# lyltc1/ZebraPose

Measured on AMD Instinct MI355X. Metric: 256x256 crops/sec (R34 DeepLabv3 inference bs=32, forward + code->vertex decode), higher is better.
Workload: dtype f32; 1 GPU; configs[1]: ResNet34+DeepLabv3 inference bs=32 on 1xMI355X, synthetic 256x256 crops, 16-bit code head, on-device decode; model=BinaryCodeNet_Deeplab(34, 16, 2, concat=True), global_batch=32, per_gpu_batch=32, input=256x256, parallelism=replicas1, precision=fp32, launch=hipgraph, fp32_engine=two-plane fp16 split fp32 (ZP_F32H2; range-guarded, full-range x3 fallback), correspondences_last_step=227718

## Files before the change

zebrapose_amd/csrc/zp_conv.hip:

```cpp
#include <type_traits>
#include "zp_common.h"
#include "zp_conv_kern.h"
#include "zp_conv3.h"

namespace zp {

__device__ uint4 g_zero_page[8];

template <typename T, int WC, int WP, int NWP, bool BNR = false>
__device__ __forceinline__ void conv_epilogue(const zp_conv_args& A, const zp_conv_sub& S, f32x4 (&acc)[WC][WP],
                                              const int p0, const int c0, const int wc, const int wp, const int lane,
                                              const int M, const int GHW, const int bx, const int zi,
                                              const int nz, unsigned* rflag = nullptr, float* red = nullptr) {
  int pn[WP], poy[WP], pox[WP];
  bool pok[WP];
  {
    const int pw0 = p0 + wp * 16 * WP + (lane & 15);
    int n = pw0 / GHW, rr = pw0 - n * GHW;
    int gy = rr / A.GW, gx = rr - gy * A.GW;
    const bool fast = A.GW % 16 == 0;
#pragma unroll
    for (int j = 0; j < WP; ++j) {
      const int p = pw0 + j * 16;
      pok[j] = p < M;
// ... 1975 lines not shown
}

extern "C" long long zp_conv2d_split_ws(const zp_conv_args* a) {
  if (!a || (a->dtype != ZP_F32X3 && a->dtype != ZP_F32H2)) return 0;
  const int ns = conv3_nsplit(*a);
  return ns > 1 ? (long long)ns * a->nsub * a->N * a->GH * a->GW * a->Cout * 4 : 0;
}

extern "C" int zp_conv_tuning(int key, int value) {
  int* g = nullptr;
  switch (key) {
    case 0: g = &g_tc256_min_blocks; break;
    case 1: g = &g_conv_flags; break;
    case 2: g = &g_strip_c64; break;
    case 6: g = &g_quad_min_blocks; break;
    case 3:
    case 4:
    case 5: return wgrad_tuning(key, value);
    case 7: return conv3_strip_mode(value);
    case 8: return conv3_min_blocks(value);
    case 9: return conv3_splitk_mode(value);
    case 10: return conv3w_mode(value);
    case 11: return conv3w_min_blocks(value);
    case 12: return conv3w_splitk_mode(value);
    case 13: return conv3w_acc_mode(value);
    case 14: return conv3w_tp128_mode(value);
    case 15: return bn_fused_mode(value);
    case 16: return conv3_subint_mode(value);
    case 17: return conv3w_subint_mode(value);
    case 18: return conv3w_mf32_mode(value);
    case 19: return conv3_pipe_st_mode(value);
    case 20: return stem_wgs_mode(value);
    case 21: return conv3w_pfb_mode(value);
    default: return -1;
  }
  const int old = *g;
  *g = value;
  return old;
}
```

zebrapose_amd/csrc/zp_conv3.h:

```cpp
#pragma once
#include "zp_common.h"

namespace zp {
int conv3_tc(const zp_conv_args& a);
int conv3_tp(const zp_conv_args& a, int tc);
bool conv3_strip_ok(const zp_conv_args& a, int tc);
int conv3_strip_mode(int v);
int conv3_min_blocks(int v);
int conv3_splitk_mode(int v);
int conv3_nsplit(const zp_conv_args& a);
int conv3_subint_mode(int v);
int conv3_pipe_st_mode(int v);
int stem_wgs_mode(int v);
int conv3w_pfb_mode(int v);
int wgrad_tuning(int key, int v);
int conv3_launch(const zp_conv_args& a, hipStream_t st, int flags, const zp_head_args* head = nullptr);
struct conv_taps;
bool conv3w_ok(const zp_conv_args& a);
int conv3w_mode(int v);
int conv3w_min_blocks(int v);
void conv3w_launch(const zp_conv_args& a, const conv_taps& tg, hipStream_t st, int flags, float* ws, int nsplit);
int conv3w_splitk(const zp_conv_args& a);
int conv3w_splitk_mode(int v);
int conv3w_tp(const zp_conv_args& a);
int conv3w_tp_head(const zp_conv_args& a);
int conv3w_acc_mode(int v);
int conv3w_tp128_mode(int v);
int conv3w_subint_mode(int v);
int conv3w_mf32_mode(int v);
bool conv3w_mf32_on();
void conv3w32_launch(const zp_conv_args& a, const conv_taps& tg, hipStream_t st, int flags, bool str);
void conv3w_head_launch(const zp_conv_args& a, const conv_taps& tg, const zp_head_args& h, hipStream_t st, int flags);
}
```

zebrapose_amd/csrc/zp_conv3.hip:

```cpp
#include <stdlib.h>
#include "zp_conv_kern.h"
#include "zp_conv3.h"

namespace zp {

__device__ __forceinline__ void block_barrier() {
  __builtin_amdgcn_s_barrier();
  asm volatile("" ::: "memory");
}

template <int NPL, int WC, int WP>
__device__ __forceinline__ void conv3_epilogue(const zp_conv_args& A, const zp_conv_sub& S, f32x4 (&acc)[WC][WP],
                                               const int p0, const int c0, const int wc, const int wp,
                                               const int lane, const int M, const int GHW, const int flags,
                                               unsigned* rflag) {
  using SP = SplitF32<NPL>;
  const int lr = lane & 15;
  bool bad = false;
  int pn[WP], poy[WP], pox[WP];
  bool pok[WP];
#pragma unroll
  for (int j = 0; j < WP; ++j) {
    const int p = p0 + wp * 16 * WP + j * 16 + lr;
    pok[j] = p < M;
    const int pp = pok[j] ? p : 0;
    const int n = pp / GHW, rr = pp - n * GHW;
    const int gy = rr / A.GW, gx = rr - gy * A.GW;
    pn[j] = n;
    poy[j] = gy * S.oys + S.oyo;
    pox[j] = gx * S.oxs + S.oxo;
  }
  const long psy = (long)A.N * S.OH * S.OW * S.ldy;
  const long psr = (long)A.N * S.OH * S.OW * A.ldr;
  if constexpr (WC % 2 == 0) {
    const bool paired = A.out_mode == ZP_OUT_NHWC && S.ldy % 8 == 0 && S.cy0 % 8 == 0 && A.Cout % 32 == 0 &&
// ... 315 lines not shown
  static_assert(WP == 4 || WP == 8, "pixel fragments per wave");
  __shared__ uint4 lds[ST * UNITS * 64];
  static_assert(ST * UNITS * 1024 <= 160 * 1024, "LDS");
  static_assert(((NPL - 1) * NT + WC + 3) * 1024 < 65536, "ds_read immediate range");
  int tb = (int)blockIdx.z / nsplit;
  const int kz = (int)blockIdx.z - tb * nsplit;
  const int tid = threadIdx.x, lane = tid & 63;
  const int wid = __builtin_amdgcn_readfirstlane(tid >> 6);
  const int wc = wid / NWP, wp = wid % NWP;
  const int GHW = A.GH * A.GW;
  const int M = A.N * GHW;
  int bx = blockIdx.x, by = blockIdx.y;
  const int total = gridDim.x * gridDim.y;
  if ((flags & 1048576) && nsplit == 1 && A.nsub > 1 && (total & 7) == 0) {
    const int gid = blockIdx.x + gridDim.x * (blockIdx.y + gridDim.y * blockIdx.z);
    const int q = gid >> 3;
    tb = q % A.nsub;
    const int tile = (gid & 7) * (total >> 3) + q / A.nsub;
    bx = tile / gridDim.y;
    by = tile - bx * gridDim.y;
  } else if (flags & 2) {
    const int bid = blockIdx.x + gridDim.x * blockIdx.y;
    const int lin = (total & 7) ? bid : (bid & 7) * (total >> 3) + (bid >> 3);
    bx = lin / gridDim.y;
    by = lin - bx * gridDim.y;
  }
  tb = __builtin_amdgcn_readfirstlane(tb);
  const zp_conv_sub& S = A.sub[tb];
  const int p0 = bx * TP, c0 = by * TC;
  const int CB = A.Cin / 32;
  const int ny = TG.ny[tb], nx = TG.nx[tb], dty = TG.dty[tb], dtx = TG.dtx[tb];
  const int nK_all = S.ntaps * CB;
  const int ks0 = (int)((long)kz * nK_all / nsplit);
  const int nK = (int)((long)(kz + 1) * nK_all / nsplit) - ks0;
  const int lr = lane & 15, lk = (lane >> 4) * 8;
  const unsigned psx_b = (unsigned)((long)A.N * A.IH * A.IW * A.ldx * 2);
  const unsigned psw_b = (unsigned)((long)A.w_rows * A.k_pad * 2);

  unsigned ubase[TPW], uym[TPW], uxm[TPW];
#pragma unroll
  for (int k = 0; k < TPW; ++k) {
    const int t = wid + NW * k;
    ubase[k] = 0u;
    uym[k] = uxm[k] = 0u;
    if (t >= NT) continue;
    if (t < NTW) {
      ubase[k] = (unsigned)(((long)(c0 + t * 16 + lr) * A.k_pad + lk) * 2);
    } else {
      const int m = p0 + (t - NTW) * 16 + lr;
      const bool ok = m < M;
      const int mm = ok ? m : 0;
      const int n = mm / GHW, rr = mm - n * GHW;
      const int gy = rr / A.GW, gx = rr - gy * A.GW;
      const int y0 = gy * A.sy, x0 = gx * A.sx;
      ubase[k] = (unsigned)(((((long)n * A.IH + y0) * A.IW + x0) * A.ldx + A.cx0 + lk) * 2);
      unsigned ym = 0, xm = 0;
      for (int q = 0; q < ny; ++q) ym |= (unsigned)((unsigned)(y0 + TG.ty0[tb] + q * dty) < (unsigned)A.IH) << q;
      for (int q = 0; q < nx; ++q) xm |= (unsigned)((unsigned)(x0 + TG.tx0[tb] + q * dtx) < (unsigned)A.IW) << q;
      uym[k] = ok ? ym : 0u;
      uxm[k] = xm;
    }
  }
#if defined(__HIP_DEVICE_COMPILE__)
  const __amdgpu_buffer_rsrc_t xrsrc = __builtin_amdgcn_make_buffer_rsrc((void*)A.x, (short)0, (int)TG.x_bytes, 0x00020000);
  const __amdgpu_buffer_rsrc_t wrsrc = __builtin_amdgcn_make_buffer_rsrc((void*)S.w, (short)0, (int)TG.w_bytes[tb], 0x00020000);
#endif
  int w_cb = ks0 / S.ntaps, w_t = ks0 - (ks0 / S.ntaps) * S.ntaps;
  int w_tyi = w_t / nx, w_txi = w_t - (w_t / nx) * nx;
  const int step_x = dtx * A.ldx * 2, step_y = dty * A.IW * A.ldx * 2;
  int act_off = ((TG.ty0[tb] * A.IW + TG.tx0[tb]) * A.ldx) * 2 + w_tyi * step_y + w_txi * step_x + w_cb * 64;
  int w_koff = (w_t * A.Cin + w_cb * 32) * 2;
  const int cin2 = A.Cin * 2;
  const bool abl_dma = flags & 4096, abl_mfma = flags & 8192;
  auto issue = [&](int ks, int stage) {
    unsigned voff[TPW];
#pragma unroll
    for (int k = 0; k < TPW; ++k) {
      const bool w = wid + NW * k < NTW;
      const bool ok = (uym[k] >> w_tyi) & (uxm[k] >> w_txi) & 1u;
      voff[k] = w ? ubase[k] : (ok ? ubase[k] + (unsigned)act_off : 0x80000000u);
    }
#if defined(__HIP_DEVICE_COMPILE__)
#pragma unroll
    for (int k = 0; k < TPW; ++k) {
      const int t = wid + NW * k;
      if (t >= NT) continue;
#pragma unroll
      for (int pl = 0; pl < NPL; ++pl) {
        auto* d = (__attribute__((address_space(3))) void*)&lds[(stage * UNITS + pl * NT + t) * 64];
        if (t < NTW) __builtin_amdgcn_raw_ptr_buffer_load_lds(wrsrc, d, 16, voff[k], pl * psw_b + w_koff, 0, 0);
        else __builtin_amdgcn_raw_ptr_buffer_load_lds(xrsrc, d, 16, voff[k], pl * psx_b, 0, 0);
      }
    }
#endif
    (void)ks;
    ++w_t;
    w_koff += cin2;
    act_off += step_x;
    if (++w_txi == nx) {
      w_txi = 0;
      act_off += step_y - nx * step_x;
      if (++w_tyi == ny) {
        w_tyi = 0;
        w_t = 0;
        ++w_cb;
        act_off += 64 - ny * step_y;
        w_koff = w_cb * 64;
      }
    }
  };

  constexpr int A2C = PIPE ? WC : 1, A2P = PIPE ? WP : 1;
  f32x4 acc[WC][WP], acc2[A2C][A2P];
#pragma unroll
  for (int i = 0; i < WC; ++i)
#pragma unroll
    for (int j = 0; j < WP; ++j) acc[i][j] = (f32x4){0.f, 0.f, 0.f, 0.f};
#pragma unroll
  for (int i = 0; i < A2C; ++i)
#pragma unroll
    for (int j = 0; j < A2P; ++j) acc2[i][j] = (f32x4){0.f, 0.f, 0.f, 0.f};

  const unsigned l0 = lds_addr(lds) + (unsigned)lane * 16u;
  unsigned abase[ST], bbase[ST];
#pragma unroll
  for (int s = 0; s < ST; ++s) {
    abase[s] = l0 + (unsigned)(s * UNITS + wc * WC) * 1024u;
    bbase[s] = l0 + (unsigned)(s * UNITS + NTW + wp * WP) * 1024u;
  }
  const int awo = (wc * WC) * 64 + lane, bwo = (NTW + wp * WP) * 64 + lane;
  auto read_a = [&](auto s_c, uint4 (&af)[NPL][WC]) {
    constexpr int s = decltype(s_c)::value;
    static_for<NPL>([&](auto p_c) {
      constexpr int p = decltype(p_c)::value;
      static_for<WC>([&](auto i) {
        if constexpr (PIPE) af[p][i] = lds[(s * UNITS + p * NT + i) * 64 + awo];
        else af[p][i] = ds_read16<(p * NT + i) * 1024>(abase[s]);
      });
    });
  };
  auto read_b = [&](auto s_c, auto j0_c, auto j1_c, uint4 (&bfr)[NPL][WP]) {
    constexpr int s = decltype(s_c)::value, J0 = decltype(j0_c)::value, J1 = decltype(j1_c)::value;
// ... 66 lines not shown
      constexpr int s = decltype(s_c)::value;
      const bool more = ks + ST - 1 < nK;
      if (more && !abl_dma) issue(ks + ST - 1, (s + ST - 1) % ST);
      uint4 af[NPL][WC], bfr[NPL][WP];
      read_a(s_c, af);
      read_b(s_c, J0c{}, JHc{}, bfr);
      asm volatile("s_waitcnt lgkmcnt(0)" ::: "memory");
      __builtin_amdgcn_sched_barrier(0);
      read_b(s_c, JHc{}, JWc{}, bfr);
      auto wait_next = [&]() {
        if (more && !abl_dma) vm_wait<GRP * (ST - 2)>();
        else vm_wait<0>();
      };
      if (pingpong) {
        wait_next();
        block_barrier();
        __builtin_amdgcn_sched_barrier(0);
      }
      if (flags & 4) __builtin_amdgcn_s_setprio(1);
      mfmas_part(J0c{}, JHc{}, af, bfr);
      __builtin_amdgcn_sched_barrier(0);
      asm volatile("s_waitcnt lgkmcnt(0)" ::: "memory");
      __builtin_amdgcn_sched_barrier(0);
      mfmas_part(JHc{}, JWc{}, af, bfr);
      __builtin_amdgcn_sched_barrier(0);
      if (flags & 4) __builtin_amdgcn_s_setprio(0);
      if (!pingpong) wait_next();
      block_barrier();
      __builtin_amdgcn_sched_barrier(0);
    };
    using I0 = std::integral_constant<int, 0>;
    using I1 = std::integral_constant<int, 1>;
    using I2 = std::integral_constant<int, 2>;
    issue(0, 0);
    if (ST == 3 && nK > 1) {
      issue(1, 1);
      vm_wait<GRP>();
    } else {
      vm_wait<0>();
    }
    block_barrier();
    __builtin_amdgcn_sched_barrier(0);
    if (pingpong && wid >= 4) block_barrier();
    if constexpr (ST == 3) {
      for (int ks = 0; ks < nK; ks += 3) {
        step(I0{}, ks);
        if (ks + 1 >= nK) break;
        step(I1{}, ks + 1);
        if (ks + 2 >= nK) break;
        step(I2{}, ks + 2);
      }
    } else {
      for (int ks = 0; ks < nK; ks += 2) {
        step(I0{}, ks);
        if (ks + 1 >= nK) break;
        step(I1{}, ks + 1);
      }
    }
    if (pingpong && wid < 4) block_barrier();
  } else {
    uint4 fa0[NPL][WC], fb0[NPL][WP], fa1[NPL][WC], fb1[NPL][WP];
    int issued = 0;
    for (int q = 0; q < ST; ++q)
      if (q < nK) {
        issue(q, q);
        ++issued;
      }
// ... 358 lines not shown
    sg->W = W;
    sg->TR = TR;
    sg->SW = SW;
    sg->SR = SR;
    sg->ty0 = ty0;
    sg->dty = dty;
    sg->tx0 = tx0;
    sg->dtx = dtx;
    sg->pad = pad;
  }
  return true;
}

static int g_splitk = 1;
static int g_subint = -1;
int conv3_subint_mode(int v) {
  const int old = g_subint;
  g_subint = v;
  return old;
}

static int g_pipe_st = -1;
int conv3_pipe_st_mode(int v) {
  const int old = g_pipe_st;
  g_pipe_st = v;
  return old;
}
static int conv3_pipe_st() {
  static const int env = getenv("ZP_CONV3_PIPE_ST") ? atoi(getenv("ZP_CONV3_PIPE_ST")) : 2;
  const int v = g_pipe_st >= 0 ? g_pipe_st : env;
  return v == 3 || v == 4 ? v : 2;
}

int conv3_splitk_mode(int v) {
  const int old = g_splitk;
  g_splitk = v;
  return old;
}

int conv3_nsplit(const zp_conv_args& a) {
  if (!g_splitk || a.out_mode != ZP_OUT_NHWC || a.nsub < 1) return 1;
  const int tc = conv3_tc(a);
  if (tc == 256) return conv3w_splitk(a);
  const long blocks = (long)ceil_div((long)a.N * a.GH * a.GW, conv3_tp(a, tc)) * ceil_div(a.Cout, tc) * a.nsub;
  int nK = 1 << 30;
  for (int s = 0; s < a.nsub; ++s) nK = min(nK, a.sub[s].ntaps * (a.Cin / 32));
  if (blocks >= 256) return 1;
  int ns = 1;
  while (ns < 16 && blocks * ns * 2 <= 512 && nK / (ns * 2) >= (a.nsub > 1 ? 4 : 8)) ns *= 2;
  return ns;
}

template <int NPL>
static void conv3_dispatch(const zp_conv_args& a, const conv_taps& tg, int tc, hipStream_t st, int fl) {
  if (tc == 256) {
    const int ns = a.stats ? conv3w_splitk(a) : 1;
    conv3w_launch(a, tg, st, fl, (float*)a.stats, ns);
    if (ns > 1) {
      const long total = (long)a.N * a.GH * a.GW * ((a.Cout + 3) / 4);
      const int blocks = (int)(total + 255) / 256 < 8192 ? (int)((total + 255) / 256) : 8192;
      hipLaunchKernelGGL((k_splitk_epi<NPL>), dim3(blocks, a.nsub), dim3(256), 0, st, a, (const float*)a.stats, ns,
                         tg.rflag);
    }
    return;
  }
  const int ns = a.stats ? conv3_nsplit(a) : 1;
// ... 48 lines not shown
  }
}

int conv3_launch(const zp_conv_args& a, hipStream_t st, int fl, const zp_head_args* head) {
  const int npl = a.dtype == ZP_F32H2 ? 2 : 3;
  ZP_CHECK_ARG(a.Cin > 0 && a.Cin % 32 == 0, "zp_conv2d: split fp32 needs Cin %% 32 == 0 (got %d; the stem runs in f32 "
               "with out_mode ZP_OUT_NHWC_X3 / _H2)", a.Cin);
  ZP_CHECK_ARG(a.ldx >= a.cx0 + a.Cin && a.cx0 % 8 == 0 && a.ldx % 8 == 0, "zp_conv2d: bad ldx/cx0");
  ZP_CHECK_ARG(a.k_pad % 32 == 0, "zp_conv2d: k_pad %d not a multiple of 32", a.k_pad);
  ZP_CHECK_ARG(a.out_mode == ZP_OUT_NHWC || a.out_mode == ZP_OUT_HEAD_NCHW,
               "zp_conv2d: split fp32 writes split NHWC (ZP_OUT_NHWC) or the f32 head (ZP_OUT_HEAD_NCHW)");
  const int tc = conv3_tc(a);
  ZP_CHECK_ARG(a.w_rows % tc == 0 && a.w_rows >= a.Cout, "zp_conv2d: w_rows %d", a.w_rows);
  for (int s = 0; s < a.nsub; ++s) {
    const zp_conv_sub& S = a.sub[s];
    ZP_CHECK_ARG(S.w && S.y, "zp_conv2d: sub %d null w/y", s);
    ZP_CHECK_ARG(S.ntaps >= 1 && S.ntaps <= ZP_MAX_TAPS && (long)S.ntaps * a.Cin <= a.k_pad,
                 "zp_conv2d: sub %d ntaps %d / k_pad %d", s, S.ntaps, a.k_pad);
    if (a.out_mode == ZP_OUT_NHWC)
      ZP_CHECK_ARG(S.ldy >= S.cy0 + a.Cout && S.cy0 % 4 == 0 && S.ldy % 4 == 0, "zp_conv2d: bad ldy/cy0");
    else
      ZP_CHECK_ARG(S.y2 || a.Cout == 1, "zp_conv2d: head needs y2");
    ZP_CHECK_ARG(S.OH == a.sub[0].OH && S.OW == a.sub[0].OW, "zp_conv2d: split-fp32 subs must share the output shape");
  }
  if (a.res) ZP_CHECK_ARG(a.ldr >= a.cr0 + a.Cout && a.cr0 % 4 == 0 && a.ldr % 4 == 0, "zp_conv2d: bad residual ld");
  conv_taps tg{};
  const long long xb = (long long)npl * a.N * a.IH * a.IW * a.ldx * 2;
  const long long wb = (long long)npl * a.w_rows * a.k_pad * 2;
  ZP_CHECK_ARG(xb < (1ll << 31) && wb < (1ll << 31),
               "zp_conv2d: split input (%lld B) / weights (%lld B) must stay below 2 GiB per launch (split the batch)",
               xb, wb);
  tg.x_bytes = (unsigned)xb;
  tg.rflag = npl == 2 ? range_flag() : nullptr;
  for (int s = 0; s < a.nsub; ++s) {
    const zp_conv_sub& S = a.sub[s];
    tg.w_bytes[s] = (unsigned)wb;
    int nx = 1;
    while (nx < S.ntaps && S.ty[nx] == S.ty[0]) ++nx;
    const int ny = S.ntaps / nx;
    tg.ny[s] = ny;
    tg.nx[s] = nx;
    tg.ty0[s] = S.ty[0];
    tg.tx0[s] = S.tx[0];
    tg.dty[s] = ny > 1 ? S.ty[nx] - S.ty[0] : 0;
    tg.dtx[s] = nx > 1 ? S.tx[1] - S.tx[0] : 0;
    bool grid = ny * nx == S.ntaps && ny <= 32 && nx <= 32;
    for (int t = 0; grid && t < S.ntaps; ++t)
      grid = S.ty[t] == tg.ty0[s] + (t / nx) * tg.dty[s] && S.tx[t] == tg.tx0[s] + (t % nx) * tg.dtx[s];
    ZP_CHECK_ARG(grid, "zp_conv2d: sub %d taps must form a (row x column) grid of at most 32 x 32, rows outer", s);
  }
  if (head) {
    const zp_head_args& h = *head;
    ZP_CHECK_ARG(tc == 256 && a.Cout == 256 && a.nsub == 1 && npl == 2,
                 "zp_conv2d_head: not a fused-head geometry (zp_conv2d_head_ok)");
    ZP_CHECK_ARG(h.w && h.mask && (h.code || h.cout == 1) && h.cout >= 1 && h.cout <= 32, "zp_conv2d_head: bad head");
    ZP_CHECK_ARG(h.C2 >= 0 && h.C2 % 32 == 0 && h.k_pad % 8 == 0 && h.k_pad >= a.Cout + h.C2 && h.k_pad <= 504,
                 "zp_conv2d_head: C2 %d / k_pad %d", h.C2, h.k_pad);
    ZP_CHECK_ARG(h.C2 == 0 || (h.x2 && h.ldx2 % 8 == 0 && h.cx20 % 8 == 0 && h.ldx2 >= h.cx20 + h.C2),
                 "zp_conv2d_head: x2 layout");
    conv3w_head_launch(a, tg, h, st, fl);
    ZP_LAUNCH_CHECK("zp_conv2d_head");
    return ZP_OK;
  }
  if (npl == 2) conv3_dispatch<2>(a, tg, tc, st, fl);
  else conv3_dispatch<3>(a, tg, tc, st, fl);
  ZP_LAUNCH_CHECK("zp_conv2d split-f32");
  return ZP_OK;
}


bool conv3_strip_ok(const zp_conv_args& a, int tc) { return conv3_strip(a, tc, nullptr); }

}
```

zebrapose_amd/csrc/zp_conv3w.hip:

```cpp
#include "zp_conv_kern.h"
#include "zp_conv3.h"

namespace zp {

constexpr int ACC_FLUSH = 0;
constexpr int ACC_SA = 1;
constexpr int ACC_PS = 2;
constexpr int ACC_FS = 3;
constexpr int ACC_P2 = 4;

__device__ __forceinline__ void wbarrier() {
  __builtin_amdgcn_s_barrier();
  asm volatile("" ::: "memory");
}

#ifdef ZP_STAMP
constexpr int ZP_STAMP_WAVES = 1 << 17;
__device__ unsigned long long zp_stamp_buf[ZP_STAMP_WAVES * 8];
#endif

template <int ABL, int DM, bool HEAD, bool SGB = false, bool PF = false, bool BF = false, bool STR = false,
          int NUM = ACC_FLUSH, int TPX = 256, bool PFB = false>
__global__ void __launch_bounds__(512) k_conv3w(const zp_conv_args A, const conv_taps TG, const int flags,
                                                const zp_head_args H, float* __restrict__ ws, const int nsplit) {
  constexpr int NPL = 2;
  constexpr int TC = 256, TP = TPX;
  static_assert(TP == 256 || TP == 128, "pixel tile");
  static_assert(TP == 256 || (!HEAD && !BF && DM == 1), "the 256 x 128 tile: plain epilogue, default DMA order");
  constexpr bool SA = NUM == ACC_SA || NUM == ACC_PS || NUM == ACC_FS;
  constexpr bool P2 = NUM == ACC_P2;
  static_assert(!P2 || (TPX == 128 && !HEAD), "the persistent correction accumulator: 256 x 128 tiles");
  static_assert(!PFB || (STR && !P2 && NUM == ACC_FLUSH && TPX == 256), "pixel-fragment prefetch: the strip tile");
  constexpr int NTW = TC / 16, NT = (TC + TP) / 16;
  constexpr int UNITS = NPL * NT;
// ... 9 lines not shown
  __shared__ uint4 lds[LDSU * 64];
  static_assert(LDSU * 1024 <= 160 * 1024, "LDS");
  static_assert(((NPL - 1) * NT + NT - 1) * 1024 < 65536, "ds_read immediate range");
  int tb = (int)blockIdx.z / nsplit;
  const int kz = (int)blockIdx.z - tb * nsplit;
  const int tid = threadIdx.x, lane = tid & 63;
  const int wid = __builtin_amdgcn_readfirstlane(tid >> 6);
  const int wc = wid >> 2, wp = wid & 3;
  const int GHW = A.GH * A.GW;
  const int M = A.N * GHW;
  int bx = blockIdx.x, by = blockIdx.y;
  const int total = gridDim.x * gridDim.y;
  if ((flags & 32768) && nsplit == 1 && A.nsub > 1 && (total & 7) == 0) {
    const int gid = blockIdx.x + gridDim.x * (blockIdx.y + gridDim.y * blockIdx.z);
    const int q = gid >> 3;
    tb = q % A.nsub;
    const int tile = (gid & 7) * (total >> 3) + q / A.nsub;
    bx = tile / gridDim.y;
    by = tile - bx * gridDim.y;
  } else if (flags & 2) {
    const int bid = blockIdx.x + gridDim.x * blockIdx.y;
    const int lin = (total & 7) ? bid : (bid & 7) * (total >> 3) + (bid >> 3);
    bx = lin / gridDim.y;
    by = lin - bx * gridDim.y;
  }
  tb = __builtin_amdgcn_readfirstlane(tb);
  const zp_conv_sub& S = A.sub[tb];
  const int p0 = bx * TP, c0 = by * TC;
  const int CB = A.Cin / 32;
  const int ny = TG.ny[tb], nx = TG.nx[tb], dty = TG.dty[tb], dtx = TG.dtx[tb];
  const int nK_all = S.ntaps * CB;
  const int kq = STR ? nx : 1, nq = nK_all / kq;
  const int ks0 = (int)((long)kz * nq / nsplit) * kq;
  const int nK = (int)((long)(kz + 1) * nq / nsplit) * kq - ks0;
  const int lr = lane & 15, lk = (lane >> 4) * 8;
  const unsigned psx_b = (unsigned)((long)A.N * A.IH * A.IW * A.ldx * 2);
  const unsigned psw_b = (unsigned)((long)A.w_rows * A.k_pad * 2);

  unsigned ubase[TPW], uym[TPW], uxm[TPW];
#pragma unroll
  for (int k = 0; k < TPW; ++k) {
    const int t = wid + 8 * k;
    uym[k] = uxm[k] = 0u;
    if (t < NTW) {
      ubase[k] = (unsigned)(((long)(c0 + t * 16 + lr) * A.k_pad + lk) * 2);
    } else {
      const int m = p0 + (t - NTW) * 16 + lr;
      const bool ok = m < M;
      const int mm = ok ? m : 0;
      const int n = mm / GHW, rr = mm - n * GHW;
      const int gy = rr / A.GW, gx = rr - gy * A.GW;
      const int y0 = gy * A.sy, x0 = gx * A.sx;
      ubase[k] = (unsigned)(((((long)n * A.IH + y0) * A.IW + x0) * A.ldx + A.cx0 + lk) * 2);
      unsigned ym = 0, xm = 0;
      for (int q = 0; q < ny; ++q) ym |= (unsigned)((unsigned)(y0 + TG.ty0[tb] + q * dty) < (unsigned)A.IH) << q;
      for (int q = 0; q < nx; ++q) xm |= (unsigned)((unsigned)(x0 + TG.tx0[tb] + q * dtx) < (unsigned)A.IW) << q;
      uym[k] = ok ? ym : 0u;
      uxm[k] = xm;
    }
  }
  int nsp = 16, SW = 0, sh0 = 0;
  unsigned sbase[3], sym[3];
  int sj[WP];
  if constexpr (STR) {
    const int sx0 = min(TG.tx0[tb], TG.tx0[tb] + (nx - 1) * dtx);
    sh0 = TG.tx0[tb] - sx0;
    SW = A.GW + (nx - 1) * (dtx < 0 ? -dtx : dtx);
    const int TR = TP / A.GW;
    nsp = (TR * SW + 15) >> 4;
    const int n = p0 / GHW, oy0 = (p0 - n * GHW) / A.GW;
#pragma unroll
    for (int k = 0; k < 3; ++k) {
      const int sp = (wid + 8 * k) * 16 + lr;
      const int r = sp / SW, c = sp - (sp / SW) * SW;
      const int ix = c + sx0, iyb = oy0 + r + TG.ty0[tb];
      unsigned ym = 0;
      for (int q = 0; q < ny; ++q) ym |= (unsigned)((unsigned)(iyb + q * dty) < (unsigned)A.IH) << q;
      sym[k] = (r < TR && (unsigned)ix < (unsigned)A.IW) ? ym : 0u;
      sbase[k] = (unsigned)(((((long)n * A.IH + iyb) * A.IW + ix) * A.ldx + A.cx0 + lk) * 2);
    }
#pragma unroll
    for (int j = 0; j < WP; ++j) {
      const int q = wp * 16 * WP + j * 16 + lr;
      sj[j] = (q / A.GW) * SW + q % A.GW;
    }
  }
#if defined(__HIP_DEVICE_COMPILE__)
  const __amdgpu_buffer_rsrc_t xrsrc = __builtin_amdgcn_make_buffer_rsrc((void*)A.x, (short)0, (int)TG.x_bytes, 0x00020000);
  const __amdgpu_buffer_rsrc_t wrsrc = __builtin_amdgcn_make_buffer_rsrc((void*)S.w, (short)0, (int)TG.w_bytes[tb], 0x00020000);
#endif
  const int t0 = ks0 % S.ntaps;
  int w_cb = ks0 / S.ntaps, w_tyi = t0 / nx, w_txi = t0 - (t0 / nx) * nx;
  const int step_x = dtx * A.ldx * 2, step_y = dty * A.IW * A.ldx * 2;
  int act_off = ((TG.ty0[tb] * A.IW + TG.tx0[tb]) * A.ldx) * 2 + w_tyi * step_y + w_txi * step_x + w_cb * 64;
  int w_koff = (t0 * A.Cin + w_cb * 32) * 2;
  const int cin2 = A.Cin * 2;
  struct DmaStep {
    unsigned voff[TPW];
    int koff;
  };
  unsigned pf_sink = 0;
  const bool pf_hi = (lane >> 5) & 1;
  constexpr int PFT = TPW - 1;
  const unsigned pf_base = pf_hi ? ubase[PFT] : ubase[2], pf_ym = pf_hi ? uym[PFT] : uym[2], pf_xm = pf_hi ? uxm[PFT] : uxm[2];
  const unsigned pf_plane = ((lane >> 4) & 1) ? psx_b : 0u;
  auto prep = [&](DmaStep& d) {
#pragma unroll
    for (int k = 0; k < TPW; ++k) {
      bool ok = (uym[k] >> w_tyi) & (uxm[k] >> w_txi) & 1u;
      if constexpr (ABL == 6) ok = ok && w_txi == 0;
      d.voff[k] = k < 2 ? ubase[k] : (ok ? ubase[k] + (unsigned)act_off : 0x80000000u);
    }
#if defined(__HIP_DEVICE_COMPILE__)
    if constexpr (PF) {
      const bool ok = w_tyi == 0 && w_txi == 0 && w_cb + 1 < CB && (pf_ym & pf_xm & 1u);
      const unsigned vo = ok ? pf_base + (unsigned)(act_off + 64) + pf_plane : 0x80000000u;
      pf_sink = __builtin_amdgcn_raw_buffer_load_b32(xrsrc, vo, 0, 0);
    }
#endif
    d.koff = w_koff;
    w_koff += cin2;
    act_off += step_x;
    if (++w_txi == nx) {
      w_txi = 0;
      act_off += step_y - nx * step_x;
      if (++w_tyi == ny) {
        w_tyi = 0;
        ++w_cb;
        act_off += 64 - ny * step_y;
        w_koff = w_cb * 64;
      }
    }
  };
  auto piece = [&](auto q_c, int stage, const DmaStep& d) {
    constexpr int q = decltype(q_c)::value, k = q / 2, pl = q % 2;
    if constexpr ((ABL == 4 && k < 2) || (ABL == 5 && k >= 2)) return;
    if constexpr (STR && k >= 2) return;
    const int t = wid + 8 * k;
#if defined(__HIP_DEVICE_COMPILE__)
    auto* dst = (__attribute__((address_space(3))) void*)&lds[(stage * ASTG + pl * APL + t) * 64];
    if constexpr (k < 2) __builtin_amdgcn_raw_ptr_buffer_load_lds(wrsrc, dst, 16, d.voff[k], pl * psw_b + d.koff, 0, 0);
    else __builtin_amdgcn_raw_ptr_buffer_load_lds(xrsrc, dst, 16, d.voff[k], pl * psx_b, 0, 0);
#else
    (void)t; (void)stage; (void)d;
#endif
  };
  auto issue = [&](int stage) {
    DmaStep d;
    prep(d);
    static_for<2 * TPW>([&](auto q_c) { piece(q_c, stage, d); });
  };
  int g_cb = ks0 / S.ntaps, g_tyi = (ks0 - (ks0 / S.ntaps) * S.ntaps) / nx;
  auto strip_issue = [&](int gst) {
    const unsigned goff = (unsigned)(g_tyi * step_y + g_cb * 64);
    static_for<3>([&](auto k_c) {
      constexpr int k = decltype(k_c)::value;
      const int P = wid + 8 * k;
      if (k < 2 || P < nsp) {
        const unsigned vo = ((sym[k] >> g_tyi) & 1u) ? sbase[k] + goff : 0x80000000u;
#if defined(__HIP_DEVICE_COMPILE__)
#pragma unroll
        for (int pl = 0; pl < NPL; ++pl) {
          auto* dst = (__attribute__((address_space(3))) void*)&lds[(2 * ASTG + (gst * NPL + pl) * SPMAX + P) * 64];
          __builtin_amdgcn_raw_ptr_buffer_load_lds(xrsrc, dst, 16, vo, pl * psx_b, 0, 0);
// ... 178 lines not shown
        } else {
          MT::mma(acc[i][j], af[i % 3][0], bf[0][j]);
        }
      }
      if constexpr (NUM == ACC_PS) flush(acc[i], c2);
      if constexpr ((NUM == ACC_FLUSH || NUM == ACC_FS) && i > 0) flush(acc[i - 1], c2p);
      if constexpr (NUM == ACC_FLUSH || NUM == ACC_FS) {
#pragma unroll
        for (int j = 0; j < WP; ++j) c2p[j] = c2[j];
      }
      if constexpr (SGB) {
        static_for<4>([&](auto) {
          __builtin_amdgcn_sched_group_barrier(0x008, 2, 0);
          __builtin_amdgcn_sched_group_barrier(0x002, 1, 0);
        });
        __builtin_amdgcn_sched_group_barrier(0x008, 4, 0);
      }
      __builtin_amdgcn_sched_barrier(0);
    });
    if constexpr (NUM == ACC_FLUSH || NUM == ACC_FS) flush(acc[WC - 1], c2p);
    ZP_STAMP_AT(1);
    if constexpr (PFB) {
      int ntxi = r_txi + 1, ngs = r_gs;
      if (ntxi == nx) {
        ntxi = 0;
        ngs ^= 1;
      }
      __builtin_amdgcn_sched_barrier(0);
      load_bf(ngs, ntxi);
      __builtin_amdgcn_sched_barrier(0);
    }
  };

  issue(0);
  if constexpr (STR) strip_issue(0);
  vm_wait<0>();
  wbarrier();
  __builtin_amdgcn_sched_barrier(0);
  if constexpr (PFB) load_bf(r_gs, r_txi);
  using I0 = std::integral_constant<int, 0>;
  using I1 = std::integral_constant<int, 1>;
  if (flags & 65536) {
    if (wid >= 4) __builtin_amdgcn_s_setprio(1);
  }
  auto end_step = [&](const bool sn) {
    if (STR && sn && nx > 1) vm_wait<4>();
    else vm_wait<0>();
    asm volatile("" ::"v"(pf_sink));
    ZP_STAMP_AT(2);
    if constexpr (!abl_bar) wbarrier();
    __builtin_amdgcn_sched_barrier(0);
    ZP_STAMP_AT(3);
    if constexpr (STR) {
      if (++r_txi == nx) {
        r_txi = 0;
        r_gs ^= 1;
      }
    }
  };
  if constexpr (P2) {
    for (int ks = 0; ks < nK; ++ks) {
      const bool sn = STR && r_txi == 0 && ks + nx < nK;
      step(ks & 1, ks + 1 < nK, sn);
      end_step(sn);
    }
  } else {
#ifdef ZP_STAMP
// ... 378 lines not shown
#endif
static int g_conv3w_pfb = -1;
int conv3w_pfb_mode(int v) {
  const int old = g_conv3w_pfb;
  g_conv3w_pfb = v;
  return old;
}
static bool conv3w_pfb_on() {
  static const int env = getenv("ZP_CONV3W_PFB") ? atoi(getenv("ZP_CONV3W_PFB")) : 1;
  return (g_conv3w_pfb >= 0 ? g_conv3w_pfb : env) != 0;
}
void conv3w_launch(const zp_conv_args& a0, const conv_taps& tg0, hipStream_t st, int fl, float* ws, int ns) {
  zp_conv_args a = a0;
  conv_taps tg = tg0;
  if (a.nsub > 1 && !(fl & 134217728)) {
    int ord[ZP_MAX_SUB];
    for (int s = 0; s < a.nsub; ++s) ord[s] = s;
    for (int i = 1; i < a.nsub; ++i)
      for (int j = i; j > 0 && a0.sub[ord[j]].ntaps > a0.sub[ord[j - 1]].ntaps; --j) {
        const int t = ord[j];
        ord[j] = ord[j - 1];
        ord[j - 1] = t;
      }
    for (int s = 0; s < a.nsub; ++s) {
      const int o = ord[s];
      a.sub[s] = a0.sub[o];
      tg.ny[s] = tg0.ny[o];
      tg.nx[s] = tg0.nx[o];
      tg.ty0[s] = tg0.ty0[o];
      tg.dty[s] = tg0.dty[o];
      tg.tx0[s] = tg0.tx0[o];
      tg.dtx[s] = tg0.dtx[o];
      tg.w_bytes[s] = tg0.w_bytes[o];
    }
  }
  const zp_head_args H{};
  const int acc = (fl & 536870912) ? ACC_FLUSH : conv3w_acc();
  if (a.nsub > 1 && ns == 1 && conv3w_subint()) fl |= 32768;
  const bool str = conv3w_strip_ok(a, tg, fl, ns);
  if (ns == 1 && conv3w_tp(a) == 128) {
    const dim3 g128((unsigned)(((long)a.N * a.GH * a.GW + 127) / 128), (unsigned)(a.Cout / 256), (unsigned)a.nsub);
    const bool s128 = conv3w_strip_ok(a, tg, fl, ns, 128);
    if (acc == ACC_P2) {
      if (s128) hipLaunchKernelGGL((k_conv3w<0, 1, false, false, false, false, true, ACC_P2, 128>), g128, dim3(512), 0, st, a, tg, fl, H, ws, ns);
      else hipLaunchKernelGGL((k_conv3w<0, 1, false, false, false, false, false, ACC_P2, 128>), g128, dim3(512), 0, st, a, tg, fl, H, ws, ns);
    } else if (s128) {
      hipLaunchKernelGGL((k_conv3w<0, 1, false, false, false, false, true, ACC_FLUSH, 128>), g128, dim3(512), 0, st, a, tg, fl, H, ws, ns);
    } else {
      hipLaunchKernelGGL((k_conv3w<0, 1, false, false, false, false, false, ACC_FLUSH, 128>), g128, dim3(512), 0, st, a, tg, fl, H, ws, ns);
    }
    return;
  }
  if (ns == 1 && acc == ACC_FLUSH && conv3w_mf32_on()) {
    conv3w32_launch(a, tg, st, fl, str);
    return;
  }
  const dim3 grid((unsigned)(((long)a.N * a.GH * a.GW + 255) / 256), (unsigned)(a.Cout / 256), (unsigned)(a.nsub * ns));
  if (fl & 4096) hipLaunchKernelGGL((k_conv3w<1, 1, false>), grid, dim3(512), 0, st, a, tg, fl, H, ws, ns);
  else if (fl & 8192) hipLaunchKernelGGL((k_conv3w<2, 1, false>), grid, dim3(512), 0, st, a, tg, fl, H, ws, ns);
  else if (fl & 131072) hipLaunchKernelGGL((k_conv3w<3, 1, false>), grid, dim3(512), 0, st, a, tg, fl, H, ws, ns);
  else if (fl & 4194304) hipLaunchKernelGGL((k_conv3w<4, 1, false>), grid, dim3(512), 0, st, a, tg, fl, H, ws, ns);
  else if (fl & 8388608) hipLaunchKernelGGL((k_conv3w<5, 1, false>), grid, dim3(512), 0, st, a, tg, fl, H, ws, ns);
  else if (fl & 262144) hipLaunchKernelGGL((k_conv3w<0, 2, false>), grid, dim3(512), 0, st, a, tg, fl, H, ws, ns);
  else if (fl & 524288) hipLaunchKernelGGL((k_conv3w<0, 8, false>), grid, dim3(512), 0, st, a, tg, fl, H, ws, ns);
  else if (fl & 1048576) {
    if (str) hipLaunchKernelGGL((k_conv3w<0, 1, false, true, false, false, true>), grid, dim3(512), 0, st, a, tg, fl, H, ws, ns);
// ... 41 lines not shown
```

zebrapose_amd/csrc/zp_conv_kern.h:

```cpp
#pragma once
#include <type_traits>
#include "zp_common.h"

#ifndef ZP_ABL
#define ZP_ABL 0
#endif

namespace zp {

template <typename T> struct MfmaTraits;
template <> struct MfmaTraits<bf16_t> {
  static constexpr int E = 8;
  static __device__ __forceinline__ void mma(f32x4& acc, const uint4& a, const uint4& b) {
    acc = __builtin_amdgcn_mfma_f32_16x16x32_bf16(__builtin_bit_cast(bf16x8, a), __builtin_bit_cast(bf16x8, b),
                                                  acc, 0, 0, 0);
  }
};
template <> struct MfmaTraits<f16_t> {
  static constexpr int E = 8;
  static __device__ __forceinline__ void mma(f32x4& acc, const uint4& a, const uint4& b) {
    acc = __builtin_amdgcn_mfma_f32_16x16x32_f16(__builtin_bit_cast(f16x8, a), __builtin_bit_cast(f16x8, b),
                                                 acc, 0, 0, 0);
  }
};
template <> struct MfmaTraits<float> {
  static constexpr int E = 4;
  static __device__ __forceinline__ void mma(f32x4& acc, const uint4& a, const uint4& b) {
    acc = __builtin_amdgcn_mfma_f32_16x16x4f32(__uint_as_float(a.x), __uint_as_float(b.x), acc, 0, 0, 0);
    acc = __builtin_amdgcn_mfma_f32_16x16x4f32(__uint_as_float(a.y), __uint_as_float(b.y), acc, 0, 0, 0);
    acc = __builtin_amdgcn_mfma_f32_16x16x4f32(__uint_as_float(a.z), __uint_as_float(b.z), acc, 0, 0, 0);
    acc = __builtin_amdgcn_mfma_f32_16x16x4f32(__uint_as_float(a.w), __uint_as_float(b.w), acc, 0, 0, 0);
  }
};

__device__ __forceinline__ int swz(int row, int chunk) { return row * 8 + (chunk ^ (row & 7)); }


template <int N>
__device__ __forceinline__ void vm_wait() {
  static_assert(N >= 0 && N < 64, "vmcnt range");
  asm volatile("s_waitcnt vmcnt(%0)" ::"n"(N) : "memory");
}

struct conv_taps {
  int ny[ZP_MAX_SUB], nx[ZP_MAX_SUB], ty0[ZP_MAX_SUB], dty[ZP_MAX_SUB], tx0[ZP_MAX_SUB], dtx[ZP_MAX_SUB];
  unsigned x_bytes, w_bytes[ZP_MAX_SUB];
  unsigned* rflag;
};

__device__ __forceinline__ unsigned lds_addr(const void* p) {
  return (unsigned)(uintptr_t)(const __attribute__((address_space(3))) void*)p;
}

template <int OFF>
__device__ __forceinline__ uint4 ds_read16(unsigned addr) {
  static_assert(OFF >= 0 && OFF < 65536, "ds offset range");
  uint4 r;
  asm volatile("ds_read_b128 %0, %1 offset:%2" : "=v"(r) : "v"(addr), "n"(OFF) : "memory");
  return r;
}

__device__ __forceinline__ uint4 scale_hi(const uint4 a) {
  typedef _Float16 h2v __attribute__((ext_vector_type(2)));
  const h2v k = {(_Float16)2048.f, (_Float16)2048.f};
  uint4 r;
  r.x = __builtin_bit_cast(unsigned, __builtin_bit_cast(h2v, a.x) * k);
  r.y = __builtin_bit_cast(unsigned, __builtin_bit_cast(h2v, a.y) * k);
  r.z = __builtin_bit_cast(unsigned, __builtin_bit_cast(h2v, a.z) * k);
  r.w = __builtin_bit_cast(unsigned, __builtin_bit_cast(h2v, a.w) * k);
  return r;
}

template <int N, typename F, int I = 0>
__device__ __forceinline__ void static_for(F&& f) {
  if constexpr (I < N) {
    f(std::integral_constant<int, I>{});
    static_for<N, F, I + 1>(static_cast<F&&>(f));
  }
}

// ... 10 lines not shown
```

Measured before the change: 3449 crops/s.

## Skip conv taps that are fully out-of-bounds for an output tile

Adds per-tile live-tap masks so the 3x3 conv kernels skip K-steps whose filter taps fall entirely in padding for every output pixel of the tile, shrinking nK and the DMA/MFMA work. A host-side check enables this only for sub-convolutions where dead taps can occur, and it defaults on. The cost is extra scalar setup, a while loop to advance the tap iterator, and the risk of mishandled split-K boundaries. Strided-strip variants are excluded.

```diff
diff --git a/zebrapose_amd/csrc/zp_conv.hip b/zebrapose_amd/csrc/zp_conv.hip
--- a/zebrapose_amd/csrc/zp_conv.hip
+++ b/zebrapose_amd/csrc/zp_conv.hip
@@ -2031,6 +2031,7 @@
     case 19: return conv3_pipe_st_mode(value);
     case 20: return stem_wgs_mode(value);
     case 21: return conv3w_pfb_mode(value);
+    case 22: return conv3_tap_skip_mode(value);
     default: return -1;
   }
   const int old = *g;
diff --git a/zebrapose_amd/csrc/zp_conv3.h b/zebrapose_amd/csrc/zp_conv3.h
--- a/zebrapose_amd/csrc/zp_conv3.h
+++ b/zebrapose_amd/csrc/zp_conv3.h
@@ -13,6 +13,7 @@
 int conv3_pipe_st_mode(int v);
 int stem_wgs_mode(int v);
 int conv3w_pfb_mode(int v);
+int conv3_tap_skip_mode(int v);
 int wgrad_tuning(int key, int v);
 int conv3_launch(const zp_conv_args& a, hipStream_t st, int flags, const zp_head_args* head = nullptr);
 struct conv_taps;
diff --git a/zebrapose_amd/csrc/zp_conv3.hip b/zebrapose_amd/csrc/zp_conv3.hip
--- a/zebrapose_amd/csrc/zp_conv3.hip
+++ b/zebrapose_amd/csrc/zp_conv3.hip
@@ -1,6 +1,7 @@
 #include <stdlib.h>
 #include "zp_conv_kern.h"
 #include "zp_conv3.h"
+#include "zp_tap_live.h"
 
 namespace zp {
 
@@ -382,7 +383,19 @@
   const int ny = TG.ny[tb], nx = TG.nx[tb], dty = TG.dty[tb], dtx = TG.dtx[tb];
   const int nK_all = S.ntaps * CB;
   const int ks0 = (int)((long)kz * nK_all / nsplit);
-  const int nK = (int)((long)(kz + 1) * nK_all / nsplit) - ks0;
+  const int ke0 = (int)((long)(kz + 1) * nK_all / nsplit);
+  tap_live LV;
+  LV.rows = ny >= 32 ? ~0u : (1u << ny) - 1u;
+  LV.cols = nx >= 32 ? ~0u : (1u << nx) - 1u;
+  const bool skip = (TG.skip >> tb) & 1;
+  if (skip)
+    LV = tap_live_masks(p0, p0 + TP, M, A.GH, A.GW, A.IH, A.IW, A.sy, A.sx, TG.ty0[tb], TG.tx0[tb], dty, dtx, ny, nx);
+  const unsigned lrows = (unsigned)__builtin_amdgcn_readfirstlane((int)LV.rows);
+  const unsigned lcols = (unsigned)__builtin_amdgcn_readfirstlane((int)LV.cols);
+  LV.rows = lrows;
+  LV.cols = lcols;
+  const int nK = !skip ? ke0 - ks0
+                       : __builtin_amdgcn_readfirstlane(tap_live_before(LV, ny, nx, ke0) - tap_live_before(LV, ny, nx, ks0));
   const int lr = lane & 15, lk = (lane >> 4) * 8;
   const unsigned psx_b = (unsigned)((long)A.N * A.IH * A.IW * A.ldx * 2);
   const unsigned psw_b = (unsigned)((long)A.w_rows * A.k_pad * 2);
@@ -422,28 +435,7 @@
   int w_koff = (w_t * A.Cin + w_cb * 32) * 2;
   const int cin2 = A.Cin * 2;
   const bool abl_dma = flags & 4096, abl_mfma = flags & 8192;
-  auto issue = [&](int ks, int stage) {
-    unsigned voff[TPW];
-#pragma unroll
-    for (int k = 0; k < TPW; ++k) {
-      const bool w = wid + NW * k < NTW;
-      const bool ok = (uym[k] >> w_tyi) & (uxm[k] >> w_txi) & 1u;
-      voff[k] = w ? ubase[k] : (ok ? ubase[k] + (unsigned)act_off : 0x80000000u);
-    }
-#if defined(__HIP_DEVICE_COMPILE__)
-#pragma unroll
-    for (int k = 0; k < TPW; ++k) {
-      const int t = wid + NW * k;
-      if (t >= NT) continue;
-#pragma unroll
-      for (int pl = 0; pl < NPL; ++pl) {
-        auto* d = (__attribute__((address_space(3))) void*)&lds[(stage * UNITS + pl * NT + t) * 64];
-        if (t < NTW) __builtin_amdgcn_raw_ptr_buffer_load_lds(wrsrc, d, 16, voff[k], pl * psw_b + w_koff, 0, 0);
-        else __builtin_amdgcn_raw_ptr_buffer_load_lds(xrsrc, d, 16, voff[k], pl * psx_b, 0, 0);
-      }
-    }
-#endif
-    (void)ks;
+  auto advance = [&]() {
     ++w_t;
     w_koff += cin2;
     act_off += step_x;
@@ -458,6 +450,37 @@
         w_koff = w_cb * 64;
       }
     }
+  };
+  auto to_live = [&]() {
+    while (!((lrows >> w_tyi) & (lcols >> w_txi) & 1u)) advance();
+  };
+  if (nK > 0) to_live();
+  int w_left = nK;
+  auto issue = [&](int ks, int stage) {
+    unsigned voff[TPW];
+#pragma unroll
+    for (int k = 0; k < TPW; ++k) {
+      const bool w = wid + NW * k < NTW;
+      const bool ok = (uym[k] >> w_tyi) & (uxm[k] >> w_txi) & 1u;
+      voff[k] = w ? ubase[k] : (ok ? ubase[k] + (unsigned)act_off : 0x80000000u);
+    }
+#if defined(__HIP_DEVICE_COMPILE__)
+#pragma unroll
+    for (int k = 0; k < TPW; ++k) {
+      const int t = wid + NW * k;
+      if (t >= NT) continue;
+#pragma unroll
+      for (int pl = 0; pl < NPL; ++pl) {
+        auto* d = (__attribute__((address_space(3))) void*)&lds[(stage * UNITS + pl * NT + t) * 64];
+        if (t < NTW) __builtin_amdgcn_raw_ptr_buffer_load_lds(wrsrc, d, 16, voff[k], pl * psw_b + w_koff, 0, 0);
+        else __builtin_amdgcn_raw_ptr_buffer_load_lds(xrsrc, d, 16, voff[k], pl * psx_b, 0, 0);
+      }
+    }
+#endif
+    (void)ks;
+    (void)w_koff;
+    advance();
+    if (--w_left > 0) to_live();
   };
 
   constexpr int A2C = PIPE ? WC : 1, A2P = PIPE ? WP : 1;
@@ -590,7 +613,7 @@
     using I0 = std::integral_constant<int, 0>;
     using I1 = std::integral_constant<int, 1>;
     using I2 = std::integral_constant<int, 2>;
-    issue(0, 0);
+    if (nK > 0) issue(0, 0);
     if (ST == 3 && nK > 1) {
       issue(1, 1);
       vm_wait<GRP>();
@@ -1015,6 +1038,13 @@
   return v == 3 || v == 4 ? v : 2;
 }
 
+static int g_tap_skip = 1;
+int conv3_tap_skip_mode(int v) {
+  const int old = g_tap_skip;
+  g_tap_skip = v;
+  return old;
+}
+
 int conv3_splitk_mode(int v) {
   const int old = g_splitk;
   g_splitk = v;
@@ -1129,6 +1159,7 @@
                xb, wb);
   tg.x_bytes = (unsigned)xb;
   tg.rflag = npl == 2 ? range_flag() : nullptr;
+  tg.skip = 0;
   for (int s = 0; s < a.nsub; ++s) {
     const zp_conv_sub& S = a.sub[s];
     tg.w_bytes[s] = (unsigned)wb;
@@ -1145,6 +1176,12 @@
     for (int t = 0; grid && t < S.ntaps; ++t)
       grid = S.ty[t] == tg.ty0[s] + (t / nx) * tg.dty[s] && S.tx[t] == tg.tx0[s] + (t % nx) * tg.dtx[s];
     ZP_CHECK_ARG(grid, "zp_conv2d: sub %d taps must form a (row x column) grid of at most 32 x 32, rows outer", s);
+    const int M = a.N * a.GH * a.GW;
+    bool dead = false;
+    for (int tp = 128; tp <= 256; tp *= 2)
+      dead = dead || tap_dead_possible(tp, M, a.GH, a.GW, a.IH, a.IW, a.sy, a.sx, tg.ty0[s], tg.tx0[s], tg.dty[s],
+                                       tg.dtx[s], ny, nx);
+    if (g_tap_skip && dead) tg.skip |= 1 << s;
   }
   if (head) {
     const zp_head_args& h = *head;
diff --git a/zebrapose_amd/csrc/zp_conv3w.hip b/zebrapose_amd/csrc/zp_conv3w.hip
--- a/zebrapose_amd/csrc/zp_conv3w.hip
+++ b/zebrapose_amd/csrc/zp_conv3w.hip
@@ -1,5 +1,6 @@
 #include "zp_conv_kern.h"
 #include "zp_conv3.h"
+#include "zp_tap_live.h"
 
 namespace zp {
 
@@ -75,7 +76,19 @@
   const int nK_all = S.ntaps * CB;
   const int kq = STR ? nx : 1, nq = nK_all / kq;
   const int ks0 = (int)((long)kz * nq / nsplit) * kq;
-  const int nK = (int)((long)(kz + 1) * nq / nsplit) * kq - ks0;
+  const int ke0 = (int)((long)(kz + 1) * nq / nsplit) * kq;
+  tap_live LV;
+  LV.rows = ny >= 32 ? ~0u : (1u << ny) - 1u;
+  LV.cols = nx >= 32 ? ~0u : (1u << nx) - 1u;
+  const bool skip = !STR && ((TG.skip >> tb) & 1);
+  if (skip)
+    LV = tap_live_masks(p0, p0 + TP, M, A.GH, A.GW, A.IH, A.IW, A.sy, A.sx, TG.ty0[tb], TG.tx0[tb], dty, dtx, ny, nx);
+  const unsigned lrows = (unsigned)__builtin_amdgcn_readfirstlane((int)LV.rows);
+  const unsigned lcols = (unsigned)__builtin_amdgcn_readfirstlane((int)LV.cols);
+  LV.rows = lrows;
+  LV.cols = lcols;
+  const int nK = !skip ? ke0 - ks0
+                     : __builtin_amdgcn_readfirstlane(tap_live_before(LV, ny, nx, ke0) - tap_live_before(LV, ny, nx, ks0));
   const int lr = lane & 15, lk = (lane >> 4) * 8;
   const unsigned psx_b = (unsigned)((long)A.N * A.IH * A.IW * A.ldx * 2);
   const unsigned psw_b = (unsigned)((long)A.w_rows * A.k_pad * 2);
@@ -142,26 +155,7 @@
     unsigned voff[TPW];
     int koff;
   };
-  unsigned pf_sink = 0;
-  const bool pf_hi = (lane >> 5) & 1;
-  constexpr int PFT = TPW - 1;
-  const unsigned pf_base = pf_hi ? ubase[PFT] : ubase[2], pf_ym = pf_hi ? uym[PFT] : uym[2], pf_xm = pf_hi ? uxm[PFT] : uxm[2];
-  const unsigned pf_plane = ((lane >> 4) & 1) ? psx_b : 0u;
-  auto prep = [&](DmaStep& d) {
-#pragma unroll
-    for (int k = 0; k < TPW; ++k) {
-      bool ok = (uym[k] >> w_tyi) & (uxm[k] >> w_txi) & 1u;
-      if constexpr (ABL == 6) ok = ok && w_txi == 0;
-      d.voff[k] = k < 2 ? ubase[k] : (ok ? ubase[k] + (unsigned)act_off : 0x80000000u);
-    }
-#if defined(__HIP_DEVICE_COMPILE__)
-    if constexpr (PF) {
-      const bool ok = w_tyi == 0 && w_txi == 0 && w_cb + 1 < CB && (pf_ym & pf_xm & 1u);
-      const unsigned vo = ok ? pf_base + (unsigned)(act_off + 64) + pf_plane : 0x80000000u;
-      pf_sink = __builtin_amdgcn_raw_buffer_load_b32(xrsrc, vo, 0, 0);
-    }
-#endif
-    d.koff = w_koff;
+  auto advance = [&]() {
     w_koff += cin2;
     act_off += step_x;
     if (++w_txi == nx) {
@@ -173,6 +167,36 @@
         act_off += 64 - ny * step_y;
         w_koff = w_cb * 64;
       }
+    }
+  };
+  auto to_live = [&]() {
+    while (!((lrows >> w_tyi) & (lcols >> w_txi) & 1u)) advance();
+  };
+  if (!STR && nK > 0) to_live();
+  int w_left = nK;
+  unsigned pf_sink = 0;
+  const bool pf_hi = (lane >> 5) & 1;
+  constexpr int PFT = TPW - 1;
+  const unsigned pf_base = pf_hi ? ubase[PFT] : ubase[2], pf_ym = pf_hi ? uym[PFT] : uym[2], pf_xm = pf_hi ? uxm[PFT] : uxm[2];
+  const unsigned pf_plane = ((lane >> 4) & 1) ? psx_b : 0u;
+  auto prep = [&](DmaStep& d) {
+#pragma unroll
+    for (int k = 0; k < TPW; ++k) {
+      bool ok = (uym[k] >> w_tyi) & (uxm[k] >> w_txi) & 1u;
+      if constexpr (ABL == 6) ok = ok && w_txi == 0;
+      d.voff[k] = k < 2 ? ubase[k] : (ok ? ubase[k] + (unsigned)act_off : 0x80000000u);
+    }
+#if defined(__HIP_DEVICE_COMPILE__)
+    if constexpr (PF) {
+      const bool ok = w_tyi == 0 && w_txi == 0 && w_cb + 1 < CB && (pf_ym & pf_xm & 1u);
+      const unsigned vo = ok ? pf_base + (unsigned)(act_off + 64) + pf_plane : 0x80000000u;
+      pf_sink = __builtin_amdgcn_raw_buffer_load_b32(xrsrc, vo, 0, 0);
+    }
+#endif
+    d.koff = w_koff;
+    advance();
+    if constexpr (!STR) {
+      if (--w_left > 0) to_live();
     }
   };
   auto piece = [&](auto q_c, int stage, const DmaStep& d) {
@@ -417,7 +441,7 @@
     }
   };
 
-  issue(0);
+  if (STR || nK > 0) issue(0);
   if constexpr (STR) strip_issue(0);
   vm_wait<0>();
   wbarrier();
@@ -862,6 +886,7 @@
       tg.tx0[s] = tg0.tx0[o];
       tg.dtx[s] = tg0.dtx[o];
       tg.w_bytes[s] = tg0.w_bytes[o];
+      tg.skip = (tg.skip & ~(1 << s)) | (((tg0.skip >> o) & 1) << s);
     }
   }
   const zp_head_args H{};
diff --git a/zebrapose_amd/csrc/zp_conv_kern.h b/zebrapose_amd/csrc/zp_conv_kern.h
--- a/zebrapose_amd/csrc/zp_conv_kern.h
+++ b/zebrapose_amd/csrc/zp_conv_kern.h
@@ -46,6 +46,7 @@
   int ny[ZP_MAX_SUB], nx[ZP_MAX_SUB], ty0[ZP_MAX_SUB], dty[ZP_MAX_SUB], tx0[ZP_MAX_SUB], dtx[ZP_MAX_SUB];
   unsigned x_bytes, w_bytes[ZP_MAX_SUB];
   unsigned* rflag;
+  int skip;
 };
 
 __device__ __forceinline__ unsigned lds_addr(const void* p) {
diff --git a/zebrapose_amd/csrc/zp_tap_live.h b/zebrapose_amd/csrc/zp_tap_live.h
--- /dev/null
+++ b/zebrapose_amd/csrc/zp_tap_live.h
@@ -0,0 +1,81 @@
+#pragma once
+
+#if defined(__HIPCC__) || defined(__CUDACC__)
+#define ZP_TAP_HD __host__ __device__
+#else
+#define ZP_TAP_HD
+#endif
+
+namespace zp {
+
+struct tap_live {
+  unsigned rows, cols;
+};
+
+ZP_TAP_HD inline unsigned tap_live_axis(int ga, int gb, int s, int I, int t0, int dt, int nt) {
+  unsigned m = 0;
+  for (int q = 0; q < nt; ++q) {
+    const int off = t0 + q * dt;
+    const int gmin = off >= 0 ? 0 : s == 1 ? -off : (-off + s - 1) / s;
+    const int g = ga > gmin ? ga : gmin;
+    m |= (unsigned)(g <= gb && g * s + off <= I - 1) << q;
+  }
+  return m;
+}
+
+ZP_TAP_HD inline tap_live tap_live_masks(int p0, int p1, int M, int GH, int GW, int IH, int IW, int sy, int sx,
+                                         int ty0, int tx0, int dty, int dtx, int ny, int nx) {
+  tap_live L;
+  L.rows = L.cols = 0u;
+  if (p1 > M) p1 = M;
+  if (p0 < 0) p0 = 0;
+  if (p0 >= p1) return L;
+  const int GHW = GH * GW;
+  const int n0 = p0 / GHW, n1 = (p1 - 1) / GHW;
+  int gya = 0, gyb = GH - 1, gxa = 0, gxb = GW - 1;
+  if (n0 == n1) {
+    const int r0 = p0 - n0 * GHW, r1 = p1 - 1 - n0 * GHW;
+    gya = r0 / GW;
+    gyb = r1 / GW;
+    if (gya == gyb) {
+      gxa = r0 - gya * GW;
+      gxb = r1 - gyb * GW;
+    }
+  }
+  L.rows = tap_live_axis(gya, gyb, sy, IH, ty0, dty, ny);
+  L.cols = tap_live_axis(gxa, gxb, sx, IW, tx0, dtx, nx);
+  return L;
+}
+
+ZP_TAP_HD inline bool tap_dead_possible_axis(int gmin, int G, int s, int I, int t0, int dt, int nt) {
+  for (int q = 0; q < nt; ++q) {
+    const int off = t0 + q * dt;
+    int a = off >= 0 ? 0 : (-off + s - 1) / s;
+    if (a > G) a = G;
+    int first = I - 1 - off < 0 ? 0 : (I - 1 - off) / s + 1;
+    if (first > G) first = G;
+    const int b = G - first;
+    if (a + b >= G || a >= gmin || b >= gmin) return true;
+  }
+  return false;
+}
+ZP_TAP_HD inline bool tap_dead_possible(int TP, int M, int GH, int GW, int IH, int IW, int sy, int sx, int ty0,
+                                        int tx0, int dty, int dtx, int ny, int nx) {
+  const bool ragged = M % TP != 0 || TP < GW;
+  int rmin = ragged ? 1 : TP / GW;
+  if (rmin > GH) rmin = GH;
+  const int cmin = ragged ? 1 : GW;
+  return tap_dead_possible_axis(rmin, GH, sy, IH, ty0, dty, ny) || tap_dead_possible_axis(cmin, GW, sx, IW, tx0, dtx, nx);
+}
+
+ZP_TAP_HD inline int tap_live_popc(unsigned v) { return __builtin_popcount(v); }
+ZP_TAP_HD inline int tap_live_before(const tap_live L, int ny, int nx, int k) {
+  const int nt = ny * nx;
+  const int cb = k / nt, t = k - cb * nt;
+  const int tyi = t / nx, txi = t - tyi * nx;
+  const int pc = tap_live_popc(L.cols);
+  return cb * tap_live_popc(L.rows) * pc + tap_live_popc(L.rows & ((1u << tyi) - 1u)) * pc +
+         (int)((L.rows >> tyi) & 1u) * tap_live_popc(L.cols & ((1u << txi) - 1u));
+}
+
+}
```

New measurement: 3448 crops/s. Within noise of the previous version (-0.0%).
